# instadeepai/InstaGeo-E2E-Geospatial-ML

Hardware: AMD Instinct MI355X
Metric: HLS chips/sec (train fwd+bwd+AdamW), prithvi_eo_v1_100 224x224x6 T=1 (higher is better)
Workload: dtype bf16; 1 GPU; BASELINE.json configs[1]: Prithvi-100M fine-tune, Sen1Floods11-shaped synthetic int16 chips (6 bands, T=1, 224x224, 2 classes, weights [1,3], ignore -1, dropout 0.1); per_gpu_batch=432, global_batch=432, parallelism=dp1, launch=eager, deterministic=True

## Files before the change

instageo-e2e-geospatial-ml_amd/csrc/head.hip:

```cpp
#include "common.h"
#include "bn_fold.h"

namespace {

__device__ __forceinline__ void split_pixel(long m, long HW, long& b, long& pix) {
    if ((unsigned long)(m | HW) < (1ul << 31)) {
        const unsigned bu = (unsigned)m / (unsigned)HW;
        b = bu, pix = (long)((unsigned)m - bu * (unsigned)HW);
    } else {
        b = m / HW, pix = m - b * HW;
    }
}

template <int NV>
__device__ __forceinline__ bool ordered_grid_totals(double& t, double* __restrict__ scratch, unsigned* __restrict__ ticket) {
    static_assert(NV <= 16, "at most 16 values");
    __shared__ int s_last;
    __shared__ double s_sub[16][16];
    if (threadIdx.x < NV) scratch[(size_t)blockIdx.x * NV + threadIdx.x] = t;
    __threadfence();
    __syncthreads();
    if (threadIdx.x == 0) s_last = atomicAdd(ticket, 1u) == gridDim.x - 1;
    __syncthreads();
    if (!s_last) return false;
    __threadfence();
    const int i = threadIdx.x & 15, g = threadIdx.x >> 4;
    double a = 0.0;
    if (i < NV)
        for (unsigned b = g; b < gridDim.x; b += 16) a += *reinterpret_cast<volatile double*>(scratch + (size_t)b * NV + i);
    s_sub[g][i] = a;
    __syncthreads();
    if (threadIdx.x < NV) {
        double s = 0.0;
#pragma unroll
        for (int q = 0; q < 16; ++q) s += s_sub[q][threadIdx.x];
        t = s;
    }
    if (threadIdx.x == 0) atomicExch(ticket, 0u);
    return true;
}

constexpr int TPB = 256;
constexpr int MAXC = 16;

__device__ __forceinline__ void stage_rows(const bf16_t* __restrict__ src, char* dst, int total, int units, int pitch) {
    for (int base = threadIdx.x; base < total; base += TPB * 4) {
        uint4 b0 = make_uint4(0, 0, 0, 0), b1 = b0, b2 = b0, b3 = b0;
        const int u0 = base, u1 = base + TPB, u2 = base + 2 * TPB, u3 = base + 3 * TPB;
        if (u0 < total) b0 = *reinterpret_cast<const uint4*>(src + (size_t)u0 * 8);
        if (u1 < total) b1 = *reinterpret_cast<const uint4*>(src + (size_t)u1 * 8);
        if (u2 < total) b2 = *reinterpret_cast<const uint4*>(src + (size_t)u2 * 8);
        if (u3 < total) b3 = *reinterpret_cast<const uint4*>(src + (size_t)u3 * 8);
        if (u0 < total) *reinterpret_cast<uint4*>(dst + (u0 / units) * pitch + (u0 % units) * 16) = b0;
        if (u1 < total) *reinterpret_cast<uint4*>(dst + (u1 / units) * pitch + (u1 % units) * 16) = b1;
        if (u2 < total) *reinterpret_cast<uint4*>(dst + (u2 / units) * pitch + (u2 % units) * 16) = b2;
        if (u3 < total) *reinterpret_cast<uint4*>(dst + (u3 / units) * pitch + (u3 % units) * 16) = b3;
    }
}

__device__ __forceinline__ void stage_cols(const bf16_t* __restrict__ src, char* dst, int nrows, int units, int c0, int cu, int pitch) {
    const int total = nrows * cu;
    for (int base = threadIdx.x; base < total; base += TPB * 4) {
        uint4 b[4];
#pragma unroll
        for (int k = 0; k < 4; ++k) {
            const int u = base + k * TPB;
            b[k] = make_uint4(0, 0, 0, 0);
            if (u < total) b[k] = *reinterpret_cast<const uint4*>(src + ((size_t)(u / cu) * units + c0 + (u % cu)) * 8);
        }
#pragma unroll
        for (int k = 0; k < 4; ++k) {
            const int u = base + k * TPB;
            if (u < total) *reinterpret_cast<uint4*>(dst + (u / cu) * pitch + (u % cu) * 16) = b[k];
        }
    }
}

constexpr int CLS_CHUNK = 48;
constexpr int CLS_IG = 8;
__global__ __launch_bounds__(TPB) void classifier_fwd_kernel(const bf16_t* __restrict__ f_hi, const bf16_t* __restrict__ f_lo,
                                                             const float* __restrict__ w, const float* __restrict__ bias,
                                                             float* __restrict__ logits, long M, long HW, int C, int ncls,
                                                             uint32_t drop_seed, const uint32_t* drop_seed_dev, uint32_t drop_thresh,
                                                             float drop_inv, const float* __restrict__ bn_scale,
                                                             const float* __restrict__ bn_shift) {
    extern __shared__ __attribute__((aligned(16))) float sw[];
    if (drop_seed_dev) drop_seed += *drop_seed_dev;
    const int units = C / 8;
    const int cmax = min(units, CLS_CHUNK / 8), pitch = cmax * 16 + 16;
    const float* sbn = sw + ncls * C + ((ncls + 3) & ~3);
    char* stage = reinterpret_cast<char*>(sw + ncls * C + ((ncls + 3) & ~3) + (bn_scale ? 2 * C : 0));
    for (int i = threadIdx.x; i < ncls * C; i += TPB) sw[i] = w[i];
    for (int i = threadIdx.x; i < ncls; i += TPB) sw[ncls * C + i] = bias[i];
    if (bn_scale)
        for (int i = threadIdx.x; i < C; i += TPB) {
            sw[ncls * C + ((ncls + 3) & ~3) + i] = bn_scale[i];
            sw[ncls * C + ((ncls + 3) & ~3) + C + i] = bn_shift[i];
        }
    const long m0 = blockIdx.x * (long)TPB;
    const int npix = (int)min((long)TPB, M - m0);
    const long m = m0 + threadIdx.x;
    float acc[MAXC];
#pragma unroll
    for (int n = 0; n < MAXC; ++n) acc[n] = 0.f;
    const char* row = stage + threadIdx.x * pitch;
    for (int c0 = 0; c0 < units; c0 += cmax) {
        const int cu = min(cmax, units - c0);
        if (c0) __syncthreads();
        if (cu == units) {
            stage_rows(f_hi + (size_t)m0 * C, stage, npix * units, units, pitch);
            if (f_lo) stage_rows(f_lo + (size_t)m0 * C, stage + (size_t)TPB * pitch, npix * units, units, pitch);
        } else {
            stage_cols(f_hi + (size_t)m0 * C, stage, npix, units, c0, cu, pitch);
            if (f_lo) stage_cols(f_lo + (size_t)m0 * C, stage + (size_t)TPB * pitch, npix, units, c0, cu, pitch);
        }
        __syncthreads();
        if (m >= M) continue;
        for (int c8 = 0; c8 < cu; ++c8) {
            float f[8];
            unpack8(*reinterpret_cast<const uint4*>(row + c8 * 16), f);
            if (f_lo) {
                float g[8];
                unpack8(*reinterpret_cast<const uint4*>(row + (size_t)TPB * pitch + c8 * 16), g);
#pragma unroll
                for (int j = 0; j < 8; ++j) f[j] += g[j];
            }
            if (bn_scale) {
                const float* sc = sbn + (c0 + c8) * 8;
#pragma unroll
                for (int j = 0; j < 8; ++j) f[j] = fmaxf(fmaf(f[j], sc[j], sc[C + j]), 0.f);
            }
            if (drop_thresh) {
                const size_t idx = (size_t)m * C + (c0 + c8) * 8;
                float mk[8];
                dropout_scale4(drop_seed, (uint32_t)idx, drop_thresh, drop_inv, mk);
                dropout_scale4(drop_seed, (uint32_t)idx + 4u, drop_thresh, drop_inv, mk + 4);
#pragma unroll
                for (int j = 0; j < 8; ++j) f[j] *= mk[j];
            }
#pragma unroll
            for (int n = 0; n < MAXC; ++n) {
                if (n < ncls) {
                    const float* wr = sw + n * C + (c0 + c8) * 8;
#pragma unroll
                    for (int j = 0; j < 8; ++j) acc[n] += f[j] * wr[j];
                }
            }
        }
    }
    if (m >= M) return;
#pragma unroll
    for (int n = 0; n < MAXC; ++n)
        if (n < ncls) acc[n] += sw[ncls * C + n];
    long b, pix;
    split_pixel(m, HW, b, pix);
#pragma unroll
    for (int n = 0; n < MAXC; ++n)
        if (n < ncls) logits[(b * ncls + n) * HW + pix] = acc[n];
}

struct ClsBn {
    const float *scale, *shift, *mean, *rstd;
    double* sums;
    float* part;
    float *dgamma, *dbeta;
    double inv_n;
};

constexpr int CLS_SLAB = 8192;
template <int VEC>
__device__ __forceinline__ void cls_load(const bf16_t* hi, const bf16_t* lo, size_t idx, float* f) {
    if constexpr (VEC == 8) {
        load8_split(hi, lo, idx, f);
    } else {
        const uint2 u = *reinterpret_cast<const uint2*>(hi + idx);
        f[0] = __uint_as_float(u.x << 16), f[1] = __uint_as_float(u.x & 0xffff0000u);
        f[2] = __uint_as_float(u.y << 16), f[3] = __uint_as_float(u.y & 0xffff0000u);
        if (lo) {
            const uint2 v = *reinterpret_cast<const uint2*>(lo + idx);
            f[0] += __uint_as_float(v.x << 16), f[1] += __uint_as_float(v.x & 0xffff0000u);
            f[2] += __uint_as_float(v.y << 16), f[3] += __uint_as_float(v.y & 0xffff0000u);
        }
    }
}
template <int VEC>
__device__ __forceinline__ void cls_store(bf16_t* hi, bf16_t* lo, size_t idx, const float* f) {
    if constexpr (VEC == 8) store8_split(hi, lo, idx, f);
    else store4_split(hi, lo, idx, f);
}

template <int NC, int VEC, int MODE>
__global__ __launch_bounds__(TPB, VEC == 8 ? 1 : 2) void cls_bwd_kernel(const float* __restrict__ dl, const bf16_t* __restrict__ f_hi,
                                                         const bf16_t* __restrict__ f_lo, const float* __restrict__ w,
                                                         bf16_t* __restrict__ df_hi, bf16_t* __restrict__ df_lo, float* __restrict__ dw,
                                                         float* __restrict__ db, const double* count, long M, long HW, int C, int ncls,
                                                         uint32_t drop_seed, const uint32_t* drop_seed_dev, uint32_t drop_thresh,
                                                         float drop_inv, int iters, int ig, ClsBn bn) {
    constexpr bool HAS_BN = MODE == 1 || MODE == 2 || MODE == 5;
    constexpr bool WANT_O = MODE <= 3;
    constexpr bool WANT_DW = MODE == 0 || MODE == 1 || MODE >= 4;
    constexpr bool SFORM = MODE == 5;
    extern __shared__ __attribute__((aligned(16))) float sm[];
    unsigned long long* sdbq = reinterpret_cast<unsigned long long*>(sm);
    float* slab = sm + 32;
    float* sdl = slab + CLS_SLAB;
    if (drop_seed_dev) drop_seed += *drop_seed_dev;
    const int nu = C / VEC, nsl = TPB / nu;
    const int u = threadIdx.x % nu, sl = threadIdx.x / nu;
    const bool live = sl < nsl;
    const int c0 = u * VEC;
    const int n0 = blockIdx.y * NC;
    const int ncl = min(NC, ncls - n0);
    if (threadIdx.x < 16) sdbq[threadIdx.x] = 0ull;
    const float gscale = count ? (float)(1.0 / fmax(count[1], 1.0)) : 1.f;
    float wr[WANT_O ? NC : 1][VEC], dwa[WANT_DW ? NC : 1][VEC], s1[SFORM ? NC : 1][VEC];
#pragma unroll
    for (int n = 0; n < NC; ++n) {
#pragma unroll
        for (int j = 0; j < VEC; ++j) {
            if constexpr (WANT_O) wr[n][j] = n < ncl ? w[(size_t)(n0 + n) * C + c0 + j] : 0.f;
            if constexpr (WANT_DW) dwa[n][j] = 0.f;
            if constexpr (SFORM) s1[n][j] = 0.f;
        }
    }
    float bsc[VEC], bsh[VEC], bmu[VEC], brs[VEC], bs[VEC], bq[VEC];
    if constexpr (HAS_BN) {
#pragma unroll
        for (int j = 0; j < VEC; ++j) {
            const int c = c0 + j;
            bsc[j] = bn.scale[c], bsh[j] = bn.shift[c], bmu[j] = bn.mean[c], brs[j] = bn.rstd[c], bs[j] = 0.f, bq[j] = 0.f;
            if constexpr (MODE == 2) {
                const float k1 = (float)(bn.sums[c] * bn.inv_n), k2 = (float)(bn.sums[C + c] * bn.inv_n);
                brs[j] = bsc[j] * brs[j] * k2;
                bmu[j] = bsc[j] * k1 - bmu[j] * brs[j];
            }
        }
        if (MODE == 2 && blockIdx.x == 0)
            for (int c = threadIdx.x; c < C; c += TPB) {
                if (bn.dbeta) atomicAdd(bn.dbeta + c, (float)bn.sums[c]);
                if (bn.dgamma) atomicAdd(bn.dgamma + c, (float)bn.sums[C + c]);
            }
    }
    const long mb = (long)blockIdx.x * nsl * iters;
    const int gpx = ig * nsl;
    const size_t estep = (size_t)nsl * C;
    constexpr bool PIPE = VEC == 4 && !(MODE == 5 && NC == 16);
    constexpr int PF = PIPE ? 4 : 2;
    auto process = [&](float* f, const size_t idx, const int px) __attribute__((always_inline)) {
            float o[VEC], msk[VEC], x[VEC];
            if (drop_thresh) {
                dropout_scale4(drop_seed, (uint32_t)idx, drop_thresh, drop_inv, msk);
                if constexpr (VEC == 8) dropout_scale4(drop_seed, (uint32_t)idx + 4u, drop_thresh, drop_inv, msk + 4);
            } else {
#pragma unroll
                for (int j = 0; j < VEC; ++j) msk[j] = 1.f;
            }
            if constexpr (SFORM) {
#pragma unroll
                for (int j = 0; j < VEC; ++j) {
                    x[j] = f[j];
                    msk[j] = fmaf(x[j], bsc[j], bsh[j]) > 0.f ? msk[j] : 0.f;
                    f[j] = msk[j] * (x[j] - bmu[j]);
                }
#pragma unroll
                for (int n = 0; n < NC; ++n) {
                    const float g = sdl[n * gpx + px];
#pragma unroll
                    for (int j = 0; j < VEC; ++j) s1[n][j] = fmaf(g, msk[j], s1[n][j]), dwa[n][j] = fmaf(g, f[j], dwa[n][j]);
                }
            } else {
#pragma unroll
                for (int j = 0; j < VEC; ++j) {
                    if constexpr (HAS_BN) x[j] = f[j], f[j] = fmaxf(fmaf(x[j], bsc[j], bsh[j]), 0.f);
                    f[j] *= msk[j];
                    o[j] = 0.f;
                }
#pragma unroll
                for (int n = 0; n < NC; ++n) {
                    const float g = sdl[n * gpx + px];
#pragma unroll
                    for (int j = 0; j < VEC; ++j) {
                        if constexpr (WANT_O) o[j] = fmaf(g, wr[n][j], o[j]);
                        if constexpr (WANT_DW) dwa[n][j] = fmaf(g, f[j], dwa[n][j]);
                    }
                }
                if constexpr (WANT_O) {
#pragma unroll
                    for (int j = 0; j < VEC; ++j) o[j] *= msk[j];
                }
                if constexpr (MODE == 0 || MODE == 3) cls_store<VEC>(df_hi, df_lo, idx, o);
                if constexpr (MODE == 1) {
#pragma unroll
                    for (int j = 0; j < VEC; ++j) {
                        const float dyr = fmaf(x[j], bsc[j], bsh[j]) > 0.f ? o[j] : 0.f;
                        bs[j] += dyr;
                        bq[j] = fmaf(dyr, x[j] - bmu[j], bq[j]);
                    }
                }
                if constexpr (MODE == 2) {
#pragma unroll
                    for (int j = 0; j < VEC; ++j) {
                        const float dyr = fmaf(x[j], bsc[j], bsh[j]) > 0.f ? o[j] : 0.f;
                        o[j] = fmaf(bsc[j], dyr, -fmaf(brs[j], x[j], bmu[j]));
                    }
                    cls_store<VEC>(df_hi, df_lo, idx, o);
                }
            }

    };
    for (int it0 = 0; it0 < iters; it0 += ig) {
        const long mg = mb + (long)it0 * nsl;
        if (mg >= M) break;
        const int itn = min(ig, iters - it0);
        const int npx = (int)min((long)itn * nsl, M - mg);
        size_t e = (size_t)(mg + sl) * C + c0;
        float fa[PF][VEC];
        if (PIPE && live && sl < npx) {
            const int nv0 = min(itn, (npx - sl + nsl - 1) / nsl);
#pragma unroll
            for (int k = 0; k < PF; ++k) cls_load<VEC>(f_hi, f_lo, k < nv0 ? e + (size_t)k * estep : e, fa[k]);
        }
        __syncthreads();
        {
            const long b0 = mg / HW, pix0 = mg - b0 * HW;
#pragma unroll
            for (int n = 0; n < NC; ++n) {
                float part = 0.f;
                for (int px = threadIdx.x; px < gpx; px += TPB) {
                    float g = 0.f;
                    if (n < ncl && px < npx) {
                        long b = b0, pix = pix0 + px;
                        while (pix >= HW) pix -= HW, ++b;
                        g = dl[(b * ncls + n0 + n) * HW + pix] * gscale;
                    }
                    sdl[n * gpx + px] = g;
                    part += g;
                }
                if constexpr (WANT_DW) {
                    if (n < ncl) {
                        part = wave_sum(part);
                        if ((threadIdx.x & 63) == 0) {
                            if (fabsf(part) < 5.0e5f) atomicAdd(sdbq + n, (unsigned long long)__float2ll_rn(part * 17592186044416.f));
                            else ig_red_add(db + n0 + n, part);
                        }
                    }
                }
            }
        }
        __syncthreads();
        if (live) {
            const int nv = min(itn, (npx - sl + nsl - 1) / nsl);
            if constexpr (PIPE) {
                for (int t = 0; t < nv; t += PF) {
                    float fb[PF][VEC];
                    if (t + PF < nv) {
#pragma unroll
                        for (int k = 0; k < PF; ++k) cls_load<VEC>(f_hi, f_lo, t + PF + k < nv ? e + (size_t)(PF + k) * estep : e, fb[k]);
                    }
#pragma unroll
                    for (int k = 0; k < PF; ++k) {
                        if (t + k < nv) process(fa[k], e + (size_t)k * estep, (t + k) * nsl + sl);
                        __builtin_amdgcn_sched_barrier(0);
                    }
#pragma unroll
                    for (int k = 0; k < PF; ++k)
#pragma unroll
                        for (int j = 0; j < VEC; ++j) fa[k][j] = fb[k][j];
                    e += (size_t)PF * estep;
                }
            } else {
                for (int t = 0; t < nv; t += 2, e += 2 * estep) {
                    const bool two = t + 1 < nv;
                    float f[2][VEC];
                    cls_load<VEC>(f_hi, f_lo, e, f[0]);
                    cls_load<VEC>(f_hi, f_lo, two ? e + estep : e, f[1]);
#pragma unroll
                    for (int q = 0; q < 2; ++q) {
                        if (q == 1 && !two) break;
                        process(f[q], e + q * estep, (t + q) * nsl + sl);
                    }
                }
            }
        }
    }
    if constexpr (WANT_DW) {
        if constexpr (SFORM) {
#pragma unroll
            for (int n = 0; n < NC; ++n)
#pragma unroll
                for (int j = 0; j < VEC; ++j) {
                    const float wn = n < ncl ? w[(size_t)(n0 + n) * C + c0 + j] : 0.f;
                    bs[j] = fmaf(wn, s1[n][j], bs[j]);
                    bq[j] = fmaf(wn, dwa[n][j], bq[j]);
                    dwa[n][j] = fmaf(bsc[j], dwa[n][j], fmaf(bmu[j], bsc[j], bsh[j]) * s1[n][j]);
                }
        }
        const int G = max(1, min(NC, CLS_SLAB / (nsl * C)));
        for (int g0 = 0; g0 < ncl; g0 += G) {
            __syncthreads();
            if (live) {
#pragma unroll
                for (int n = 0; n < NC; ++n)
                    if (n >= g0 && n < g0 + G) {
#pragma unroll
                        for (int j = 0; j < VEC; ++j) slab[((size_t)sl * G + (n - g0)) * C + c0 + j] = dwa[n][j];
                    }
            }
            __syncthreads();
            const int nn = min(G, ncl - g0);
            for (int i = threadIdx.x; i < nn * C; i += TPB) {
                const int k = i / C, c = i - k * C;
                float t = 0.f;
                for (int s2 = 0; s2 < nsl; ++s2) t += slab[((size_t)s2 * G + k) * C + c];
                ig_red_add(dw + (size_t)(n0 + g0 + k) * C + c, t);
            }
        }
        __syncthreads();
        for (int i = threadIdx.x; i < ncl; i += TPB) ig_red_add(db + n0 + i, (float)((double)(long long)sdbq[i] * 5.684341886080802e-14));
        if constexpr (MODE == 1 || SFORM) {
            if (live) {
#pragma unroll
                for (int j = 0; j < VEC; ++j) slab[(size_t)sl * 2 * C + c0 + j] = bs[j], slab[(size_t)sl * 2 * C + C + c0 + j] = bq[j] * brs[j];
            }
            __syncthreads();
            const size_t wg = (size_t)blockIdx.y * gridDim.x + blockIdx.x;
            for (int i = threadIdx.x; i < 2 * C; i += TPB) {
                float t = 0.f;
                for (int q = 0; q < nsl; ++q) t += slab[(size_t)q * 2 * C + i];
                if (bn.part) bn.part[wg * 2 * C + i] = t;
                else atomicAdd(bn.sums + i, (double)t);
            }
        }
    }
}

struct SegArgs {
    float gamma;
    int pixel_on;
    double* parts;
    double* part;
};

template <typename LABEL, int VEC, int NCB, bool SEG>
__global__ __launch_bounds__(TPB) void ce_loss_kernel(const float* __restrict__ logits, const LABEL* __restrict__ labels,
                                                      const float* __restrict__ cw, long ignore_index, double* __restrict__ stats,
                                                      float* __restrict__ dlogits, long long* __restrict__ preds,
                                                      signed char* __restrict__ preds_i8, unsigned long long* __restrict__ confusion,
                                                      long M, long HW, int ncls, unsigned long long* __restrict__ acc, unsigned* __restrict__ arrived,
                                                      SegArgs seg) {
    extern __shared__ unsigned int hist[];
    for (int i = threadIdx.x; i < ncls * ncls; i += TPB) hist[i] = 0u;
    __syncthreads();
    float my_loss = 0.f, my_cnt = 0.f;
    unsigned cnt4[4] = {0u, 0u, 0u, 0u};
    float sP[SEG ? NCB : 1], sI[SEG ? NCB : 1];
    bool count_hist = confusion != nullptr;
    if constexpr (SEG) {
#pragma unroll
        for (int n = 0; n < NCB; ++n) sP[n] = 0.f, sI[n] = 0.f;
        count_hist = count_hist || seg.part != nullptr;
    }
    for (long m0 = (blockIdx.x * (long)TPB + threadIdx.x) * VEC; m0 < M; m0 += (long)gridDim.x * TPB * VEC) {
        long b, pix;
        split_pixel(m0, HW, b, pix);
        float z[NCB][VEC];
        LABEL lab[VEC];
#pragma unroll
        for (int n = 0; n < NCB; ++n) {
            if (n < ncls) {
                const float* src = logits + (b * ncls + n) * HW + pix;
                if constexpr (VEC == 4) {
                    const float4 v = *reinterpret_cast<const float4*>(src);
                    z[n][0] = v.x, z[n][1] = v.y, z[n][2] = v.z, z[n][3] = v.w;
                } else {
                    z[n][0] = *src;
                }
            }
        }
#pragma unroll
        for (int e = 0; e < VEC; ++e) lab[e] = labels[m0 + e];
        int amv[VEC];
#pragma unroll
        for (int e = 0; e < VEC; ++e) {
            float mx = -INFINITY;
            int am = 0;
#pragma unroll
            for (int n = 0; n < NCB; ++n)
                if (n < ncls && z[n][e] > mx) mx = z[n][e], am = n;
            const long y = (long)lab[e];
            float se = 0.f, zy = 0.f;
            [[maybe_unused]] float ey = 0.f, so = 0.f;
#pragma unroll
            for (int n = 0; n < NCB; ++n)
                if (n < ncls) {
                    if (n == (int)y) zy = z[n][e];
                    z[n][e] = expf(z[n][e] - mx);
                    se += z[n][e];
                    if constexpr (SEG) {
                        if (n == (int)y) ey = z[n][e];
                        else so += z[n][e];
                    }
                }
            const float lse0 = logf(se), rse = 1.f / se;
            const bool valid = (y != ignore_index) && y >= 0 && y < ncls;
            const float w0 = valid ? (cw ? cw[y] : 1.f) : 0.f;
            float wy = w0, wl = w0;
            if constexpr (SEG) {
                if (valid) {
                    if (seg.part) {
#pragma unroll
                        for (int n = 0; n < NCB; ++n)
                            if (n < ncls) {
                                const float p = z[n][e] * rse;
                                sP[n] += p;
                                sI[n] += n == (int)y ? p : 0.f;
                            }
                    }
                    if (!seg.pixel_on) {
                        wy = 0.f, wl = 0.f;
                    } else if (seg.gamma != 0.f) {
                        const float pt = ey * rse, nll = (mx - zy) + lse0;
                        const float omp = 2.f * ey < se ? 1.f - pt : so * rse;
                        const float pw = seg.gamma == 1.f ? 1.f : (seg.gamma == 2.f ? omp : powf(omp, seg.gamma - 1.f));
                        wl = w0 * (pw * omp);
                        wy = w0 * (pw * (omp + seg.gamma * pt * nll));
                    }
                }
            }
            if (valid) {
                my_loss += wl * ((mx - zy) + lse0);
                my_cnt += 1.f;
                if constexpr (NCB == 2) {
// ... 304 lines not shown
#pragma unroll
        for (int n = 0; n < MAXC; ++n)
            if (n < ncls) {
                z[n] = __expf(z[n] - mx);
                se += z[n];
            }
#pragma unroll
        for (int n = 0; n < MAXC; ++n)
            if (n < ncls) {
                float p = z[n] / se;
                p = fminf(hi, fmaxf(lo, p));
                const int bin = (int)((p - lo) / (hi - lo) * inv);
                const int idx = ((y == n ? 0 : 1) * ncls + n) * nbins + bin;
                if (USE_LDS) atomicAdd(sh + idx, 1u);
                else atomicAdd(hist + idx, 1ull);
            }
    }
    if (USE_LDS) {
        __syncthreads();
        for (int i = threadIdx.x; i < nh; i += TPB)
            if (sh[i]) atomicAdd(hist + i, (unsigned long long)sh[i]);
    }
}

__global__ __launch_bounds__(TPB) void softmax_prob_kernel(const float* __restrict__ logits, float* __restrict__ out, long M, long HW,
                                                           int ncls, int cls) {
    const long m = blockIdx.x * (long)TPB + threadIdx.x;
    if (m >= M) return;
    long b, pix;
    split_pixel(m, HW, b, pix);
    float mx = -INFINITY, zc = 0.f;
    for (int n = 0; n < ncls; ++n) mx = fmaxf(mx, logits[(b * ncls + n) * HW + pix]);
    float se = 0.f;
    for (int n = 0; n < ncls; ++n) {
        const float e = __expf(logits[(b * ncls + n) * HW + pix] - mx);
        se += e;
        if (n == cls) zc = e;
    }
    out[m] = zc / se;
}

__global__ __launch_bounds__(TPB) void mse_loss_kernel(const float* __restrict__ pred, const float* __restrict__ labels, float ignore_value,
                                                       int use_log, double* __restrict__ stats, float* __restrict__ dpred,
                                                       double* __restrict__ msums, float ee_bias, float ee_coef, int include_ee,
                                                       long M, double* __restrict__ scratch, unsigned* __restrict__ ticket) {
    __shared__ double red[TPB / 64][10];
    double a[10] = {0, 0, 0, 0, 0, 0, 0, 0, 0, 0};
    for (long m = blockIdx.x * (long)TPB + threadIdx.x; m < M; m += (long)gridDim.x * TPB) {
        const float lab = labels[m];
        const bool valid = lab != ignore_value;
        const float p = pred[m];
        const float t = use_log ? log1pf(lab) : lab;
        const float d = p - t;
        if (dpred) dpred[m] = valid ? 2.f * d : 0.f;
        if (valid) {
            a[0] += (double)(d * d);
            const float y = use_log ? expm1f(p) : p;
            const float x = use_log ? expm1f(t) : lab;
            const float e = fabsf(y - x);
            a[1] += 1.0, a[2] += x, a[3] += y, a[4] += (double)(x * y), a[5] += (double)(x * x), a[6] += (double)(y * y);
            a[7] += e, a[8] += (double)(e * e);
            if (include_ee && e <= ee_bias + ee_coef * x) a[9] += 1.0;
        }
    }
    const int lane = threadIdx.x & 63, wave = threadIdx.x >> 6;
#pragma unroll
    for (int i = 0; i < 10; ++i) {
        double v = a[i];
#pragma unroll
        for (int o = 32; o > 0; o >>= 1) v += __shfl_xor(v, o, 64);
        if (lane == 0) red[wave][i] = v;
    }
    __syncthreads();
    double t = 0.0;
    if (threadIdx.x < 10)
        for (int w = 0; w < TPB / 64; ++w) t += red[w][threadIdx.x];
    if (ordered_grid_totals<10>(t, scratch, ticket) && threadIdx.x < 10) {
        const int i = threadIdx.x;
        if (i == 0) stats[0] += t;
        else if (i == 1) {
            stats[1] += t;
            if (msums) msums[0] += t;
        } else if (msums) msums[i - 1] += t;
    }
}

__global__ __launch_bounds__(TPB) void kd_mse_loss_kernel(const float* __restrict__ pred, const float* __restrict__ teacher,
                                                          const float* __restrict__ labels, float ignore_value, int use_log,
                                                          double* __restrict__ sum, float* __restrict__ dpred, long M, double* __restrict__ scratch, unsigned* __restrict__ ticket) {
    __shared__ double red[TPB / 64];
    double a = 0.0;
    for (long m = blockIdx.x * (long)TPB + threadIdx.x; m < M; m += (long)gridDim.x * TPB) {
        if (labels[m] == ignore_value) continue;
        const float t = use_log ? log1pf(teacher[m]) : teacher[m];
        const float d = pred[m] - t;
        a += (double)(d * d);
        if (dpred) dpred[m] += 2.f * d;
    }
#pragma unroll
    for (int o = 32; o > 0; o >>= 1) a += __shfl_xor(a, o, 64);
    if ((threadIdx.x & 63) == 0) red[threadIdx.x >> 6] = a;
    __syncthreads();
    double t = 0.0;
    if (threadIdx.x == 0)
        for (int w = 0; w < TPB / 64; ++w) t += red[w];
    if (ordered_grid_totals<1>(t, scratch, ticket) && threadIdx.x == 0) *sum += t;
}

__global__ void argmax_kernel(const float* __restrict__ logits, signed char* __restrict__ out, long M, long HW, int ncls) {
    long m = blockIdx.x * (long)blockDim.x + threadIdx.x;
    if (m >= M) return;
    long b, pix;
    split_pixel(m, HW, b, pix);
    float mx = -INFINITY;
    int am = 0;
    for (int n = 0; n < ncls; ++n) {
        float z = logits[(b * ncls + n) * HW + pix];
        if (z > mx) mx = z, am = n;
    }
    out[m] = (signed char)am;
}

__global__ __launch_bounds__(TPB) void confusion_kernel(const long long* __restrict__ y_true, const long long* __restrict__ y_pred,
                                                        unsigned long long* __restrict__ confusion, long n, int k, long ignore_index,
                                                        int has_ignore) {
    extern __shared__ unsigned int hist[];
    for (int i = threadIdx.x; i < k * k; i += TPB) hist[i] = 0u;
    __syncthreads();
    for (long i = blockIdx.x * (long)TPB + threadIdx.x; i < n; i += (long)gridDim.x * TPB) {
        long long t = y_true[i], p = y_pred[i];
        if (has_ignore && t == ignore_index) continue;
        if (t < 0 || t >= k || p < 0 || p >= k) continue;
        atomicAdd(hist + (int)t * k + (int)p, 1u);
    }
    __syncthreads();
    for (int i = threadIdx.x; i < k * k; i += TPB)
        if (hist[i]) atomicAdd(confusion + i, (unsigned long long)hist[i]);
}

inline uint32_t thresh_of(float p) { return ig_drop_thresh16(p); }

}
IG_DET_TU(head)

extern "C" {

static int classifier_fwd_impl(const void* f_hi, const void* f_lo, const float* bn_scale, const float* bn_shift, const float* w,
                               const float* bias, float* logits, int B, long HW, int C, int ncls, unsigned drop_seed,
                               const unsigned* drop_seed_dev, float drop_p, void* stream) {
    IG_REQUIRE(f_hi && w && bias && logits, "ig_classifier_fwd: null pointer");
    IG_REQUIRE(C % 8 == 0 && ncls >= 1 && ncls <= MAXC, "ig_classifier_fwd: need C %% 8 == 0 and 1 <= ncls <= %d (C=%d ncls=%d)", MAXC, C, ncls);
    long M = (long)B * HW;
    if (M == 0) return IG_OK;
    const int cmax = C / 8 < CLS_CHUNK / 8 ? C / 8 : CLS_CHUNK / 8;
    size_t sm = ((size_t)ncls * C + ((ncls + 3) & ~3) + (bn_scale ? 2 * (size_t)C : 0)) * sizeof(float) + (size_t)TPB * (cmax * 16 + 16) * (f_lo ? 2 : 1);
    IG_REQUIRE(sm <= 160 * 1024, "ig_classifier_fwd: ncls x C = %d x %d weights do not fit the LDS", ncls, C);
    static bool attr_done = false;
    if (!attr_done) {
        (void)hipFuncSetAttribute((const void*)classifier_fwd_kernel, hipFuncAttributeMaxDynamicSharedMemorySize, 160 * 1024);
        attr_done = true;
    }
    hipLaunchKernelGGL(classifier_fwd_kernel, dim3((unsigned)((M + TPB - 1) / TPB)), dim3(TPB), sm, (hipStream_t)stream,
                       (const bf16_t*)f_hi, (const bf16_t*)f_lo, w, bias, logits, M, HW, C, ncls, drop_seed, drop_seed_dev, thresh_of(drop_p),
                       drop_p > 0.f ? 1.f / (1.f - drop_p) : 1.f, bn_scale, bn_shift);
    return ig_check_launch("ig_classifier_fwd");
}

int ig_classifier_fwd(const void* f_hi, const void* f_lo, const float* w, const float* bias, float* logits, int B, long HW, int C,
                      int ncls, unsigned drop_seed, const unsigned* drop_seed_dev, float drop_p, void* stream) {
    return classifier_fwd_impl(f_hi, f_lo, nullptr, nullptr, w, bias, logits, B, HW, C, ncls, drop_seed, drop_seed_dev, drop_p, stream);
}

int ig_classifier_bn_fwd(const void* x_hi, const void* x_lo, const float* scale, const float* shift, const float* w, const float* bias,
                         float* logits, int B, long HW, int C, int ncls, unsigned drop_seed, const unsigned* drop_seed_dev, float drop_p,
                         void* stream) {
    IG_REQUIRE(scale && shift, "ig_classifier_bn_fwd: null pointer");
    return classifier_fwd_impl(x_hi, x_lo, scale, shift, w, bias, logits, B, HW, C, ncls, drop_seed, drop_seed_dev, drop_p, stream);
}

static int classifier_bwd_impl(int mode, ClsBn bn, int* nwg_out, const float* dlogits, const void* f_hi, const void* f_lo, const float* w,
                               void* df_hi, void* df_lo, float* dw, float* db, const double* count, int B, long HW, int C, int ncls,
                               unsigned drop_seed, const unsigned* drop_seed_dev, float drop_p, void* stream) {
    IG_REQUIRE(dlogits && f_hi && w && (df_hi || mode == 1) && ((dw && db) || mode == 2), "ig_classifier_bwd: null pointer");
    IG_REQUIRE(C % 8 == 0 && ncls >= 1 && ncls <= MAXC, "ig_classifier_bwd: need C %% 8 == 0 and 1 <= ncls <= %d", MAXC);
    long M = (long)B * HW;
    if (M == 0) return IG_OK;
    const int nc = ncls <= 2 ? 2 : ncls <= 4 ? 4 : ncls <= 8 ? 8 : 16;
    const bool wide = ncls > 4;
    const int vec = wide ? 4 : 8;
    IG_REQUIRE(C / vec <= TPB, "ig_classifier_bwd: C must be <= %d", TPB * vec);
    const long nsl = TPB / (C / vec);
    long iters = (M + nsl * 1024 - 1) / (nsl * 1024);
    if (iters < 8) iters = 8;
    const long ppb = nsl * iters;
    const unsigned gx = (unsigned)((M + ppb - 1) / ppb);
    const unsigned gy_split = wide ? (unsigned)((ncls + 7) / 8) : 1u;
    constexpr bool one_group = true;
    if (nwg_out) {
        *nwg_out = (int)(gx * (nc == 16 && one_group ? 1u : gy_split));
        return IG_OK;
    }
    long ig = 4096 / (nc * nsl);
    const long ig_max = wide ? 32 : 8;
    ig = ig < 8 ? 8 : ig > ig_max ? ig_max : ig & ~7L;
    const size_t sm = (32 + (size_t)CLS_SLAB + (size_t)nc * ig * nsl) * sizeof(float);
    const float inv = drop_p > 0.f ? 1.f / (1.f - drop_p) : 1.f;
    constexpr bool sform = true;
#define IG_CLS_BWD(NC, VEC, MD, GY)                                                                                                      \
    do {                                                                                                                                 \
        auto kern_ = cls_bwd_kernel<NC, VEC, MD>;                                                                                        \
        static bool attr_done_ = false;                                                                                                  \
        if (!attr_done_) {                                                                                                               \
            IG_REQUIRE(hipFuncSetAttribute((const void*)kern_, hipFuncAttributeMaxDynamicSharedMemorySize, 128 << 10) == hipSuccess,     \
                       "ig_classifier_bwd: could not raise the dynamic LDS limit%s", "");                                               \
            attr_done_ = true;                                                                                                           \
        }                                                                                                                                \
        hipLaunchKernelGGL(kern_, dim3(gx, GY), dim3(TPB), sm, (hipStream_t)stream, dlogits, (const bf16_t*)f_hi,                        \
                           (const bf16_t*)f_lo, w, (bf16_t*)df_hi, (bf16_t*)df_lo, dw, db, count, M, HW, C, ncls, drop_seed,             \
                           drop_seed_dev, thresh_of(drop_p), inv, (int)iters, (int)ig, bn);                                              \
    } while (0)
#define IG_CLS_BWD_M(NC)                             \
    do {                                             \
        if (mode == 0) IG_CLS_BWD(NC, 8, 0, 1);      \
        else if (mode == 1) {                        \
            if (sform) IG_CLS_BWD(NC, 8, 5, 1);      \
            else IG_CLS_BWD(NC, 8, 1, 1);            \
        }                                            \
        else IG_CLS_BWD(NC, 8, 2, 1);                \
    } while (0)
#define IG_CLS_BWD_W(NC)                                      \
    do {                                                      \
        if (mode == 0) {                                      \
            IG_CLS_BWD(NC, 4, 3, 1);                          \
            if (NC == 16 && one_group) IG_CLS_BWD(NC, 4, 4, 1); \
            else IG_CLS_BWD(8, 4, 4, gy_split);               \
        } else if (mode == 1) {                               \
            if (NC == 16 && one_group) IG_CLS_BWD(NC, 4, 5, 1); \
            else IG_CLS_BWD(8, 4, 5, gy_split);               \
        }                                                     \
        else IG_CLS_BWD(NC, 4, 2, 1);                         \
    } while (0)
    if (nc == 2) IG_CLS_BWD_M(2);
    else if (nc == 4) IG_CLS_BWD_M(4);
    else if (nc == 8) IG_CLS_BWD_W(8);
    else IG_CLS_BWD_W(16);
#undef IG_CLS_BWD_W
#undef IG_CLS_BWD_M
#undef IG_CLS_BWD
    return ig_check_launch("ig_classifier_bwd");
}

int ig_classifier_bwd(const float* dlogits, const void* f_hi, const void* f_lo, const float* w, void* df_hi, void* df_lo, float* dw,
                      float* db, const double* count, int B, long HW, int C, int ncls, unsigned drop_seed,
                      const unsigned* drop_seed_dev, float drop_p, void* stream) {
    return classifier_bwd_impl(0, ClsBn{}, nullptr, dlogits, f_hi, f_lo, w, df_hi, df_lo, dw, db, count, B, HW, C, ncls, drop_seed,
                               drop_seed_dev, drop_p, stream);
}

int ig_classifier_bn_bwd(const float* dlogits, const void* x_hi, const void* x_lo, const float* scale, const float* shift,
                         const float* mean, const float* rstd, const float* w, void* dx_hi, void* dx_lo, float* dw, float* db,
                         float* dgamma, float* dbeta, double* sums, const double* count, int B, long HW, int C, int ncls,
                         unsigned drop_seed, const unsigned* drop_seed_dev, float drop_p, void* stream) {
    IG_REQUIRE(scale && shift && mean && rstd && sums && dx_hi, "ig_classifier_bn_bwd: null pointer");
    const long M = (long)B * HW;
    if (M == 0) return IG_OK;
    int nwg = 0;
    int rc = classifier_bwd_impl(1, ClsBn{}, &nwg, dlogits, x_hi, x_lo, w, nullptr, nullptr, dw, db, count, B, HW, C, ncls, drop_seed,
                                 drop_seed_dev, drop_p, stream);
    if (rc != IG_OK) return rc;
    ClsBn bn{scale, shift, mean, rstd, sums, nullptr, dgamma, dbeta, 1.0 / (double)M};
    if (ig_deterministic()) {
        bn.part = (float*)ig_scratch(0, (size_t)nwg * 2 * C * sizeof(float), (hipStream_t)stream);
        IG_REQUIRE(bn.part, "ig_classifier_bn_bwd: scratch allocation failed");
    } else {
        (void)hipMemsetAsync(sums, 0, 2 * (size_t)C * sizeof(double), (hipStream_t)stream);
    }
    rc = classifier_bwd_impl(1, bn, nullptr, dlogits, x_hi, x_lo, w, nullptr, nullptr, dw, db, count, B, HW, C, ncls, drop_seed,
                             drop_seed_dev, drop_p, stream);
    if (rc != IG_OK) return rc;
    if (bn.part)
        hipLaunchKernelGGL((bn_part_fold_kernel<float>), dim3(ig_cdiv(2 * C, 64)), dim3(1024), 0, (hipStream_t)stream, bn.part, sums, nwg, 2 * C);
    return classifier_bwd_impl(2, bn, nullptr, dlogits, x_hi, x_lo, w, dx_hi, dx_lo, nullptr, nullptr, count, B, HW, C, ncls, drop_seed,
                               drop_seed_dev, drop_p, stream);
}

static double* loss_scratch(unsigned** ticket, hipStream_t st) {
    double* buf = (double*)ig_scratch(2, (1024 * 16 + 2) * sizeof(double), st);
    if (!buf) return nullptr;
    *ticket = reinterpret_cast<unsigned*>(buf + 1024 * 16);
    return buf;
}

extern "C++" {
template <bool SEG>
static int ce_loss_launch(const char* who, const float* logits, const void* labels, int label_dtype, const float* class_weights, long ignore_index,
                          double* stats, float* dlogits, long long* preds, signed char* preds_i8, unsigned long long* confusion, long M, long HW,
                          int ncls, SegArgs seg, bool vec4, int nblk, void* stream) {
    size_t sm = (size_t)ncls * ncls * sizeof(unsigned);
    unsigned long long* acc_stream = nullptr;
    if (stats) {
        acc_stream = (unsigned long long*)ig_scratch(3, 4 * sizeof(unsigned long long), (hipStream_t)stream);
        if (!acc_stream) {
            ig_set_error("%s: scratch allocation failed", who);
            return IG_ERR_HIP;
        }
    }
    unsigned long long* acc = acc_stream;
    unsigned* arrived = acc ? reinterpret_cast<unsigned*>(acc + 2) : nullptr;
    dim3 grid((unsigned)nblk), block(TPB);
    hipStream_t st = (hipStream_t)stream;
#define IG_CE(LT)                                                                                                                   \
    {                                                                                                                               \
        if (vec4 && ncls <= 2)                                                                                                      \
            hipLaunchKernelGGL((ce_loss_kernel<LT, 4, 2, SEG>), grid, block, sm, st, logits, (const LT*)labels, class_weights,      \
                               ignore_index, stats, dlogits, preds, preds_i8, confusion, M, HW, ncls, acc, arrived, seg);          \
        else if (vec4)                                                                                                              \
            hipLaunchKernelGGL((ce_loss_kernel<LT, 4, 16, SEG>), grid, block, sm, st, logits, (const LT*)labels, class_weights,     \
// ... 224 lines not shown
```

Before: 5357 chips/s.

## Template classifier forward on class count and BN/lo flags, drop LDS weight staging

Specializes the classifier forward kernel on the padded class count, the BatchNorm flag and the hi/lo split flag. Weights, bias and BN parameters are now read directly from global memory instead of being copied into LDS, which shrinks shared memory so more blocks can be resident. Feature staging is merged into one chunked loader that issues all global loads before any LDS stores. Separately, the backward load loop now prefetches up to three vectors before unpacking them. The exchange is more kernel instantiations and per-element global or cached reads of the weights in the inner loop.

```diff
diff --git a/instageo-e2e-geospatial-ml_amd/csrc/head.hip b/instageo-e2e-geospatial-ml_amd/csrc/head.hip
--- a/instageo-e2e-geospatial-ml_amd/csrc/head.hip
+++ b/instageo-e2e-geospatial-ml_amd/csrc/head.hip
@@ -43,120 +43,106 @@
 constexpr int TPB = 256;
 constexpr int MAXC = 16;
 
-__device__ __forceinline__ void stage_rows(const bf16_t* __restrict__ src, char* dst, int total, int units, int pitch) {
-    for (int base = threadIdx.x; base < total; base += TPB * 4) {
-        uint4 b0 = make_uint4(0, 0, 0, 0), b1 = b0, b2 = b0, b3 = b0;
-        const int u0 = base, u1 = base + TPB, u2 = base + 2 * TPB, u3 = base + 3 * TPB;
-        if (u0 < total) b0 = *reinterpret_cast<const uint4*>(src + (size_t)u0 * 8);
-        if (u1 < total) b1 = *reinterpret_cast<const uint4*>(src + (size_t)u1 * 8);
-        if (u2 < total) b2 = *reinterpret_cast<const uint4*>(src + (size_t)u2 * 8);
-        if (u3 < total) b3 = *reinterpret_cast<const uint4*>(src + (size_t)u3 * 8);
-        if (u0 < total) *reinterpret_cast<uint4*>(dst + (u0 / units) * pitch + (u0 % units) * 16) = b0;
-        if (u1 < total) *reinterpret_cast<uint4*>(dst + (u1 / units) * pitch + (u1 % units) * 16) = b1;
-        if (u2 < total) *reinterpret_cast<uint4*>(dst + (u2 / units) * pitch + (u2 % units) * 16) = b2;
-        if (u3 < total) *reinterpret_cast<uint4*>(dst + (u3 / units) * pitch + (u3 % units) * 16) = b3;
-    }
-}
-
-__device__ __forceinline__ void stage_cols(const bf16_t* __restrict__ src, char* dst, int nrows, int units, int c0, int cu, int pitch) {
-    const int total = nrows * cu;
-    for (int base = threadIdx.x; base < total; base += TPB * 4) {
-        uint4 b[4];
-#pragma unroll
-        for (int k = 0; k < 4; ++k) {
-            const int u = base + k * TPB;
-            b[k] = make_uint4(0, 0, 0, 0);
-            if (u < total) b[k] = *reinterpret_cast<const uint4*>(src + ((size_t)(u / cu) * units + c0 + (u % cu)) * 8);
-        }
-#pragma unroll
-        for (int k = 0; k < 4; ++k) {
-            const int u = base + k * TPB;
-            if (u < total) *reinterpret_cast<uint4*>(dst + (u / cu) * pitch + (u % cu) * 16) = b[k];
-        }
-    }
-}
-
 constexpr int CLS_CHUNK = 48;
+constexpr int CLS_CU = CLS_CHUNK / 8;
 constexpr int CLS_IG = 8;
+
+template <bool LO>
+__device__ __forceinline__ void stage_chunk(const bf16_t* __restrict__ hi, const bf16_t* __restrict__ lo, char* dst, int npix, int units,
+                                            int c0, int cu, int pitch) {
+    const int q = TPB / cu, r = TPB - q * cu;
+    const int row0 = threadIdx.x / cu, col0 = threadIdx.x - row0 * cu;
+    uint4 a[CLS_CU], b[CLS_CU];
+    int row = row0, col = col0;
+#pragma unroll
+    for (int k = 0; k < CLS_CU; ++k) {
+        const bool live = k < cu && row < npix;
+        const size_t src = ((size_t)(live ? row : 0) * units + c0 + (live ? col : 0)) * 8;
+        a[k] = *reinterpret_cast<const uint4*>(hi + src);
+        if constexpr (LO) b[k] = *reinterpret_cast<const uint4*>(lo + src);
+        row += q, col += r;
+        if (col >= cu) col -= cu, ++row;
+    }
+#pragma unroll
+    for (int k = 0; k < CLS_CU; ++k) {
+        asm volatile("" ::"v"(a[k].x), "v"(a[k].y), "v"(a[k].z), "v"(a[k].w));
+        if constexpr (LO) asm volatile("" ::"v"(b[k].x), "v"(b[k].y), "v"(b[k].z), "v"(b[k].w));
+    }
+    row = row0, col = col0;
+#pragma unroll
+    for (int k = 0; k < CLS_CU; ++k) {
+        if (k < cu && row < npix) {
+            *reinterpret_cast<uint4*>(dst + row * pitch + col * 16) = a[k];
+            if constexpr (LO) *reinterpret_cast<uint4*>(dst + (size_t)TPB * pitch + row * pitch + col * 16) = b[k];
+        }
+        row += q, col += r;
+        if (col >= cu) col -= cu, ++row;
+    }
+}
+
+template <int NC, bool BN, bool LO>
 __global__ __launch_bounds__(TPB) void classifier_fwd_kernel(const bf16_t* __restrict__ f_hi, const bf16_t* __restrict__ f_lo,
                                                              const float* __restrict__ w, const float* __restrict__ bias,
                                                              float* __restrict__ logits, long M, long HW, int C, int ncls,
-                                                             uint32_t drop_seed, const uint32_t* drop_seed_dev, uint32_t drop_thresh,
+                                                             uint32_t drop_seed, const uint32_t* __restrict__ drop_seed_dev, uint32_t drop_thresh,
                                                              float drop_inv, const float* __restrict__ bn_scale,
                                                              const float* __restrict__ bn_shift) {
-    extern __shared__ __attribute__((aligned(16))) float sw[];
+    extern __shared__ __attribute__((aligned(16))) char stage[];
     if (drop_seed_dev) drop_seed += *drop_seed_dev;
     const int units = C / 8;
-    const int cmax = min(units, CLS_CHUNK / 8), pitch = cmax * 16 + 16;
-    const float* sbn = sw + ncls * C + ((ncls + 3) & ~3);
-    char* stage = reinterpret_cast<char*>(sw + ncls * C + ((ncls + 3) & ~3) + (bn_scale ? 2 * C : 0));
-    for (int i = threadIdx.x; i < ncls * C; i += TPB) sw[i] = w[i];
-    for (int i = threadIdx.x; i < ncls; i += TPB) sw[ncls * C + i] = bias[i];
-    if (bn_scale)
-        for (int i = threadIdx.x; i < C; i += TPB) {
-            sw[ncls * C + ((ncls + 3) & ~3) + i] = bn_scale[i];
-            sw[ncls * C + ((ncls + 3) & ~3) + C + i] = bn_shift[i];
-        }
+    const int cmax = min(units, CLS_CU), pitch = cmax * 16 + 16;
     const long m0 = blockIdx.x * (long)TPB;
     const int npix = (int)min((long)TPB, M - m0);
     const long m = m0 + threadIdx.x;
-    float acc[MAXC];
-#pragma unroll
-    for (int n = 0; n < MAXC; ++n) acc[n] = 0.f;
+    float acc[NC];
+#pragma unroll
+    for (int n = 0; n < NC; ++n) acc[n] = 0.f;
     const char* row = stage + threadIdx.x * pitch;
+    uint32_t idx = (uint32_t)((size_t)m * C);
     for (int c0 = 0; c0 < units; c0 += cmax) {
         const int cu = min(cmax, units - c0);
         if (c0) __syncthreads();
-        if (cu == units) {
-            stage_rows(f_hi + (size_t)m0 * C, stage, npix * units, units, pitch);
-            if (f_lo) stage_rows(f_lo + (size_t)m0 * C, stage + (size_t)TPB * pitch, npix * units, units, pitch);
-        } else {
-            stage_cols(f_hi + (size_t)m0 * C, stage, npix, units, c0, cu, pitch);
-            if (f_lo) stage_cols(f_lo + (size_t)m0 * C, stage + (size_t)TPB * pitch, npix, units, c0, cu, pitch);
-        }
+        stage_chunk<LO>(f_hi + (size_t)m0 * C, LO ? f_lo + (size_t)m0 * C : nullptr, stage, npix, units, c0, cu, pitch);
         __syncthreads();
         if (m >= M) continue;
-        for (int c8 = 0; c8 < cu; ++c8) {
+        for (int c8 = 0; c8 < cu; ++c8, idx += 8u) {
+            const int c = (c0 + c8) * 8;
             float f[8];
             unpack8(*reinterpret_cast<const uint4*>(row + c8 * 16), f);
-            if (f_lo) {
+            if constexpr (LO) {
                 float g[8];
                 unpack8(*reinterpret_cast<const uint4*>(row + (size_t)TPB * pitch + c8 * 16), g);
 #pragma unroll
                 for (int j = 0; j < 8; ++j) f[j] += g[j];
             }
-            if (bn_scale) {
-                const float* sc = sbn + (c0 + c8) * 8;
-#pragma unroll
-                for (int j = 0; j < 8; ++j) f[j] = fmaxf(fmaf(f[j], sc[j], sc[C + j]), 0.f);
+            if constexpr (BN) {
+#pragma unroll
+                for (int j = 0; j < 8; ++j) f[j] = fmaxf(fmaf(f[j], bn_scale[c + j], bn_shift[c + j]), 0.f);
             }
             if (drop_thresh) {
-                const size_t idx = (size_t)m * C + (c0 + c8) * 8;
                 float mk[8];
-                dropout_scale4(drop_seed, (uint32_t)idx, drop_thresh, drop_inv, mk);
-                dropout_scale4(drop_seed, (uint32_t)idx + 4u, drop_thresh, drop_inv, mk + 4);
+                dropout_scale4(drop_seed, idx, drop_thresh, drop_inv, mk);
+                dropout_scale4(drop_seed, idx + 4u, drop_thresh, drop_inv, mk + 4);
 #pragma unroll
                 for (int j = 0; j < 8; ++j) f[j] *= mk[j];
             }
 #pragma unroll
-            for (int n = 0; n < MAXC; ++n) {
+            for (int n = 0; n < NC; ++n) {
+#pragma clang fp contract(off)
                 if (n < ncls) {
-                    const float* wr = sw + n * C + (c0 + c8) * 8;
-#pragma unroll
-                    for (int j = 0; j < 8; ++j) acc[n] += f[j] * wr[j];
+                    const float* wr = w + (size_t)n * C + c;
+#pragma unroll
+                    for (int j = 0; j < 8; ++j) acc[n] = acc[n] + f[j] * wr[j];
                 }
             }
         }
     }
     if (m >= M) return;
-#pragma unroll
-    for (int n = 0; n < MAXC; ++n)
-        if (n < ncls) acc[n] += sw[ncls * C + n];
     long b, pix;
     split_pixel(m, HW, b, pix);
 #pragma unroll
-    for (int n = 0; n < MAXC; ++n)
-        if (n < ncls) logits[(b * ncls + n) * HW + pix] = acc[n];
+    for (int n = 0; n < NC; ++n)
+        if (n < ncls) logits[(b * ncls + n) * HW + pix] = acc[n] + bias[n];
 }
 
 struct ClsBn {
@@ -169,18 +155,31 @@
 
 constexpr int CLS_SLAB = 8192;
 template <int VEC>
-__device__ __forceinline__ void cls_load(const bf16_t* hi, const bf16_t* lo, size_t idx, float* f) {
+struct ClsRaw {
+    using T = uint4;
+};
+template <>
+struct ClsRaw<4> {
+    using T = uint2;
+};
+template <int VEC>
+__device__ __forceinline__ void cls_unpack(const typename ClsRaw<VEC>::T& u, float* f) {
     if constexpr (VEC == 8) {
-        load8_split(hi, lo, idx, f);
+        unpack8(u, f);
     } else {
-        const uint2 u = *reinterpret_cast<const uint2*>(hi + idx);
         f[0] = __uint_as_float(u.x << 16), f[1] = __uint_as_float(u.x & 0xffff0000u);
         f[2] = __uint_as_float(u.y << 16), f[3] = __uint_as_float(u.y & 0xffff0000u);
-        if (lo) {
-            const uint2 v = *reinterpret_cast<const uint2*>(lo + idx);
-            f[0] += __uint_as_float(v.x << 16), f[1] += __uint_as_float(v.x & 0xffff0000u);
-            f[2] += __uint_as_float(v.y << 16), f[3] += __uint_as_float(v.y & 0xffff0000u);
-        }
+    }
+}
+template <int VEC>
+__device__ __forceinline__ void cls_load(const bf16_t* hi, const bf16_t* lo, size_t idx, float* f) {
+    using Raw = typename ClsRaw<VEC>::T;
+    cls_unpack<VEC>(*reinterpret_cast<const Raw*>(hi + idx), f);
+    if (lo) {
+        float g[VEC];
+        cls_unpack<VEC>(*reinterpret_cast<const Raw*>(lo + idx), g);
+#pragma unroll
+        for (int j = 0; j < VEC; ++j) f[j] += g[j];
     }
 }
 template <int VEC>
@@ -369,15 +368,28 @@
                     e += (size_t)PF * estep;
                 }
             } else {
-                for (int t = 0; t < nv; t += 2, e += 2 * estep) {
-                    const bool two = t + 1 < nv;
-                    float f[2][VEC];
-                    cls_load<VEC>(f_hi, f_lo, e, f[0]);
-                    cls_load<VEC>(f_hi, f_lo, two ? e + estep : e, f[1]);
-#pragma unroll
-                    for (int q = 0; q < 2; ++q) {
-                        if (q == 1 && !two) break;
-                        process(f[q], e + q * estep, (t + q) * nsl + sl);
+                using Raw = typename ClsRaw<VEC>::T;
+                constexpr int CLS_NL = SFORM ? 3 : 2;
+                for (int t = 0; t < nv; t += CLS_NL, e += CLS_NL * estep) {
+                    Raw rh[CLS_NL], rl[CLS_NL];
+#pragma unroll
+                    for (int k = 0; k < CLS_NL; ++k) rh[k] = *reinterpret_cast<const Raw*>(f_hi + (t + k < nv ? e + k * estep : e));
+                    if (f_lo) {
+#pragma unroll
+                        for (int k = 0; k < CLS_NL; ++k) rl[k] = *reinterpret_cast<const Raw*>(f_lo + (t + k < nv ? e + k * estep : e));
+                    }
+#pragma unroll
+                    for (int k = 0; k < CLS_NL; ++k) {
+                        if (t + k >= nv) break;
+                        float f[VEC];
+                        cls_unpack<VEC>(rh[k], f);
+                        if (f_lo) {
+                            float g[VEC];
+                            cls_unpack<VEC>(rl[k], g);
+#pragma unroll
+                            for (int j = 0; j < VEC; ++j) f[j] += g[j];
+                        }
+                        process(f, e + k * estep, (t + k) * nsl + sl);
                     }
                 }
             }
@@ -988,17 +1000,28 @@
     IG_REQUIRE(C % 8 == 0 && ncls >= 1 && ncls <= MAXC, "ig_classifier_fwd: need C %% 8 == 0 and 1 <= ncls <= %d (C=%d ncls=%d)", MAXC, C, ncls);
     long M = (long)B * HW;
     if (M == 0) return IG_OK;
-    const int cmax = C / 8 < CLS_CHUNK / 8 ? C / 8 : CLS_CHUNK / 8;
-    size_t sm = ((size_t)ncls * C + ((ncls + 3) & ~3) + (bn_scale ? 2 * (size_t)C : 0)) * sizeof(float) + (size_t)TPB * (cmax * 16 + 16) * (f_lo ? 2 : 1);
-    IG_REQUIRE(sm <= 160 * 1024, "ig_classifier_fwd: ncls x C = %d x %d weights do not fit the LDS", ncls, C);
-    static bool attr_done = false;
-    if (!attr_done) {
-        (void)hipFuncSetAttribute((const void*)classifier_fwd_kernel, hipFuncAttributeMaxDynamicSharedMemorySize, 160 * 1024);
-        attr_done = true;
-    }
-    hipLaunchKernelGGL(classifier_fwd_kernel, dim3((unsigned)((M + TPB - 1) / TPB)), dim3(TPB), sm, (hipStream_t)stream,
-                       (const bf16_t*)f_hi, (const bf16_t*)f_lo, w, bias, logits, M, HW, C, ncls, drop_seed, drop_seed_dev, thresh_of(drop_p),
-                       drop_p > 0.f ? 1.f / (1.f - drop_p) : 1.f, bn_scale, bn_shift);
+    IG_REQUIRE(!bn_scale == !bn_shift, "ig_classifier_fwd: BatchNorm scale and shift come together%s", "");
+    const int cmax = C / 8 < CLS_CU ? C / 8 : CLS_CU;
+    const size_t sm = (size_t)TPB * (cmax * 16 + 16) * (f_lo ? 2 : 1);
+    const dim3 grid((unsigned)((M + TPB - 1) / TPB));
+    const float inv = drop_p > 0.f ? 1.f / (1.f - drop_p) : 1.f;
+#define IG_CLS_FWD(NC, BN, LO)                                                                                                            \
+    hipLaunchKernelGGL((classifier_fwd_kernel<NC, BN, LO>), grid, dim3(TPB), sm, (hipStream_t)stream, (const bf16_t*)f_hi,                \
+                       (const bf16_t*)f_lo, w, bias, logits, M, HW, C, ncls, drop_seed, drop_seed_dev, thresh_of(drop_p), inv, bn_scale,  \
+                       bn_shift)
+#define IG_CLS_FWD_N(NC)                             \
+    do {                                             \
+        if (bn_scale && f_lo) IG_CLS_FWD(NC, true, true);        \
+        else if (bn_scale) IG_CLS_FWD(NC, true, false);          \
+        else if (f_lo) IG_CLS_FWD(NC, false, true);              \
+        else IG_CLS_FWD(NC, false, false);                       \
+    } while (0)
+    if (ncls <= 2) IG_CLS_FWD_N(2);
+    else if (ncls <= 4) IG_CLS_FWD_N(4);
+    else if (ncls <= 8) IG_CLS_FWD_N(8);
+    else IG_CLS_FWD_N(16);
+#undef IG_CLS_FWD_N
+#undef IG_CLS_FWD
     return ig_check_launch("ig_classifier_fwd");
 }
 
```

Measured after the change: 5360 chips/s, median of 3. Within noise of the previous version (+0.1%).
